# teamtomo/torch-motion-correction

Measured on AMD Instinct MI355X. Metric: frames/sec motion-corrected, 40×4k×4k fp32 stack, 1/2/4/8 MI355X, higher is better.
Workload: dtype f32; 1 GPU; 40-frame 4096x4096 fp32 movie, global rigid shift estimate+correct (estimate_global_motion -> correct_motion, frames + sum out), 1 stack per GPU per step, consecutive steps overlapped on two HIP streams; b_factor=500

## Files before the change

torch_motion_correction_amd/csrc/mc_fft.h:

```cpp
#pragma once
#include <type_traits>
#include "mc_common.h"

__device__ __forceinline__ int lpad(int i) { return i + (i >> 4); }
__host__ __device__ constexpr int lds_len(int n) { return n + (n >> 4) + 1; }

#define MC_SQRT1_2 0.70710678118654752440f

template <int DIR>
__device__ __forceinline__ void bfly2(cfloat* a) {
  cfloat t = a[0];
  a[0] = cadd(t, a[1]);
  a[1] = csub(t, a[1]);
}

template <int DIR>
__device__ __forceinline__ void bfly4(cfloat& a0, cfloat& a1, cfloat& a2, cfloat& a3) {
  cfloat t0 = cadd(a0, a2), t1 = csub(a0, a2);
  cfloat t2 = cadd(a1, a3), t3 = cmul_i<DIR>(csub(a1, a3));
  a0 = cadd(t0, t2);
  a1 = cadd(t1, t3);
  a2 = csub(t0, t2);
  a3 = csub(t1, t3);
}

template <int DIR>
__device__ __forceinline__ void bfly8(cfloat* a) {
  bfly4<DIR>(a[0], a[2], a[4], a[6]);
  bfly4<DIR>(a[1], a[3], a[5], a[7]);
  const float c = MC_SQRT1_2;
  cfloat o1, o2, o3;
  if (DIR < 0) {
    o1 = cmake(c * (a[3].x + a[3].y), c * (a[3].y - a[3].x));
    o3 = cmake(c * (a[7].y - a[7].x), -c * (a[7].x + a[7].y));
  } else {
    o1 = cmake(c * (a[3].x - a[3].y), c * (a[3].x + a[3].y));
    o3 = cmake(-c * (a[7].x + a[7].y), c * (a[7].x - a[7].y));
  }
  o2 = cmul_i<DIR>(a[5]);
  cfloat e0 = a[0], e1 = a[2], e2 = a[4], e3 = a[6], o0 = a[1];
  a[0] = cadd(e0, o0);
  a[4] = csub(e0, o0);
  a[1] = cadd(e1, o1);
  a[5] = csub(e1, o1);
  a[2] = cadd(e2, o2);
  a[6] = csub(e2, o2);
  a[3] = cadd(e3, o3);
  a[7] = csub(e3, o3);
}

template <int R, int DIR>
__device__ __forceinline__ void bfly(cfloat* a) {
  if constexpr (R == 8) bfly8<DIR>(a);
  else if constexpr (R == 4) bfly4<DIR>(a[0], a[1], a[2], a[3]);
  else bfly2<DIR>(a);
}

template <int N>
struct FftPlan {
  static constexpr int npass() {
    int n = N, p = 0;
    while (n > 1) {
      n /= (n >= 8 ? 8 : n);
      ++p;
    }
    return p;
  }
  static constexpr int radix(int pass) {
    int n = N, r = 1;
    for (int p = 0; p <= pass; ++p) {
      r = n >= 8 ? 8 : n;
      n /= r;
    }
    return r;
  }
  static constexpr int ns(int pass) {
    int n = 1;
    for (int p = 0; p < pass; ++p) n *= radix(p);
    return n;
  }
  static constexpr int iters(int pass) { return (N / radix(pass) + MC_WG - 1) / MC_WG; }
  static constexpr int max_iters() {
    int m = 1;
    for (int p = 0; p < npass(); ++p) m = iters(p) > m ? iters(p) : m;
    return m;
  }
};

__host__ __device__ constexpr int fft_threads(int n) {
  return (n / 8) < 64 ? 64 : ((n / 8) > MC_WG ? MC_WG : (n / 8));
}

template <int N>
struct FftTwiddles {
  static constexpr int P = FftPlan<N>::npass();
  static constexpr int NT = fft_threads(N);
  static constexpr int max_iters() {
    int m = 1;
    for (int p = 0; p < P; ++p) {
      const int it = (N / FftPlan<N>::radix(p) + NT - 1) / NT;
      m = it > m ? it : m;
    }
    return m;
  }
  cfloat w[P > 1 ? P - 1 : 1][max_iters()];
  template <int DIR>
  __device__ __forceinline__ void init(int lt, const cfloat* __restrict__ tw, int tw_stride) {
#pragma unroll
    for (int p = 1; p < P; ++p) {
      const int R = FftPlan<N>::radix(p), NS = FftPlan<N>::ns(p), NB = N / R;
      const int IT = (NB + NT - 1) / NT;
#pragma unroll
      for (int it = 0; it < IT; ++it) {
        const int j = lt + it * NT;
        const int k = j & (NS - 1);
        cfloat v = tw[(j < NB ? k : 0) * (N / (NS * R)) * tw_stride];
        if (DIR > 0) v.y = -v.y;
        w[p - 1][it] = v;
      }
    }
  }
};

template <int N, int PASS, int DIR, typename Load, typename Store>
__device__ __forceinline__ void fft_pass2(int lt, const FftTwiddles<N>& T, Load load, Store store) {
  constexpr int R = FftPlan<N>::radix(PASS);
  constexpr int NS = FftPlan<N>::ns(PASS);
  constexpr int NB = N / R;
  constexpr int NT = fft_threads(N);
  constexpr int IT = (NB + NT - 1) / NT;
  cfloat v[IT][R];
#pragma unroll
  for (int it = 0; it < IT; ++it) {
    const int j = lt + it * NT;
    if (NB % NT == 0 || j < NB) {
#pragma unroll
      for (int m = 0; m < R; ++m) v[it][m] = load(j + m * NB, it, m);
      if constexpr (NS > 1) {
        const cfloat w1 = T.w[PASS - 1][it];
        v[it][1] = cmul(v[it][1], w1);
        if constexpr (R >= 4) {
          const cfloat w2 = cmul(w1, w1), w3 = cmul(w2, w1);
          v[it][2] = cmul(v[it][2], w2);
          v[it][3] = cmul(v[it][3], w3);
          if constexpr (R == 8) {
            const cfloat w4 = cmul(w2, w2), w5 = cmul(w4, w1), w6 = cmul(w3, w3), w7 = cmul(w4, w3);
            v[it][4] = cmul(v[it][4], w4);
            v[it][5] = cmul(v[it][5], w5);
            v[it][6] = cmul(v[it][6], w6);
            v[it][7] = cmul(v[it][7], w7);
          }
        }
      }
      bfly<R, DIR>(v[it]);
      const int k = j & (NS - 1);
      const int base = (j - k) * R + k;
#pragma unroll
      for (int m = 0; m < R; ++m) store(base + m * NS, v[it][m]);
    }
  }
}

template <int N, int DIR, bool LAST_TO_FUNCTOR, int PASS, typename Load, typename Store>
__device__ __forceinline__ int fft_pp_rec(cfloat* l0, cfloat* l1, int s, int lt,
                                          const FftTwiddles<N>& T, Load load, Store store) {
  constexpr int P = FftPlan<N>::npass();
  cfloat* src = ((s + PASS + 1) & 1) ? l1 : l0;
  cfloat* dst = ((s + PASS) & 1) ? l1 : l0;
  auto lds_load = [src](int i, int, int) { return src[lpad(i)]; };
  auto lds_store = [dst](int i, cfloat v) { dst[lpad(i)] = v; };
  constexpr bool LAST = (PASS == P - 1);
  if constexpr (PASS == 0 && LAST) {
    if constexpr (LAST_TO_FUNCTOR) fft_pass2<N, PASS, DIR>(lt, T, load, store);
    else { fft_pass2<N, PASS, DIR>(lt, T, load, lds_store); __syncthreads(); }
    return (s + PASS) & 1;
  } else if constexpr (PASS == 0) {
    fft_pass2<N, PASS, DIR>(lt, T, load, lds_store);
    __syncthreads();
    return fft_pp_rec<N, DIR, LAST_TO_FUNCTOR, PASS + 1>(l0, l1, s, lt, T, load, store);
  } else if constexpr (LAST) {
    if constexpr (LAST_TO_FUNCTOR) {
      fft_pass2<N, PASS, DIR>(lt, T, lds_load, store);
      return (s + PASS + 1) & 1;
    } else {
      fft_pass2<N, PASS, DIR>(lt, T, lds_load, lds_store);
      __syncthreads();
      return (s + PASS) & 1;
    }
  } else {
    fft_pass2<N, PASS, DIR>(lt, T, lds_load, lds_store);
    __syncthreads();
    return fft_pp_rec<N, DIR, LAST_TO_FUNCTOR, PASS + 1>(l0, l1, s, lt, T, load, store);
  }
}

template <int N, int DIR, bool LAST_TO_FUNCTOR, typename Load, typename Store>
__device__ __forceinline__ int wg_fft_pp(cfloat* l0, cfloat* l1, int s, int lt,
                                         const FftTwiddles<N>& T, Load load, Store store) {
  return fft_pp_rec<N, DIR, LAST_TO_FUNCTOR, 0>(l0, l1, s, lt, T, load, store);
}

template <int N, int R, int NS, int DIR, bool SYNC_MID, bool SYNC_END, typename Load, typename Store>
__device__ __forceinline__ void fft_pass(int tid, const cfloat* __restrict__ tw, int tw_stride,
                                         Load load, Store store) {
  constexpr int NB = N / R;
  constexpr int IT = (NB + MC_WG - 1) / MC_WG;
  cfloat v[IT][R];
#pragma unroll
  for (int it = 0; it < IT; ++it) {
    const int j = tid + it * MC_WG;
    if (NB >= MC_WG || j < NB) {
#pragma unroll
      for (int m = 0; m < R; ++m) v[it][m] = load(j + m * NB);
      if constexpr (NS > 1) {
        const int k = j & (NS - 1);
        cfloat w1 = tw[k * (N / (NS * R)) * tw_stride];
        if (DIR > 0) w1.y = -w1.y;
        v[it][1] = cmul(v[it][1], w1);
        if constexpr (R >= 4) {
          cfloat w2 = cmul(w1, w1), w3 = cmul(w2, w1);
          v[it][2] = cmul(v[it][2], w2);
          v[it][3] = cmul(v[it][3], w3);
          if constexpr (R == 8) {
            cfloat w4 = cmul(w2, w2), w5 = cmul(w4, w1), w6 = cmul(w3, w3), w7 = cmul(w4, w3);
            v[it][4] = cmul(v[it][4], w4);
            v[it][5] = cmul(v[it][5], w5);
            v[it][6] = cmul(v[it][6], w6);
            v[it][7] = cmul(v[it][7], w7);
          }
        }
      }
      bfly<R, DIR>(v[it]);
    }
  }
  if (SYNC_MID) __syncthreads();
#pragma unroll
  for (int it = 0; it < IT; ++it) {
    const int j = tid + it * MC_WG;
    if (NB >= MC_WG || j < NB) {
      const int k = j & (NS - 1);
      const int base = (j - k) * R + k;
#pragma unroll
      for (int m = 0; m < R; ++m) store(base + m * NS, v[it][m]);
    }
  }
  if (SYNC_END) __syncthreads();
}

template <int N, int NS, int DIR, bool FIRST, bool FIRST_LDS = false, typename Load, typename Store>
__device__ __forceinline__ void fft_rec(cfloat* line, int tid, const cfloat* __restrict__ tw,
                                        int tw_stride, Load load, Store store) {
  constexpr int REM = N / NS;
  constexpr int R = REM >= 8 ? 8 : REM;
  constexpr bool LAST = (NS * R == N);
  auto lds_load = [line](int i) { return line[lpad(i)]; };
  auto lds_store = [line](int i, cfloat v) { line[lpad(i)] = v; };
  if constexpr (FIRST && LAST) {
    fft_pass<N, R, NS, DIR, FIRST_LDS, false>(tid, tw, tw_stride, load, store);
  } else if constexpr (FIRST) {
    fft_pass<N, R, NS, DIR, FIRST_LDS, true>(tid, tw, tw_stride, load, lds_store);
    fft_rec<N, NS * R, DIR, false>(line, tid, tw, tw_stride, load, store);
  } else if constexpr (LAST) {
    fft_pass<N, R, NS, DIR, true, false>(tid, tw, tw_stride, lds_load, store);
  } else {
    fft_pass<N, R, NS, DIR, true, true>(tid, tw, tw_stride, lds_load, lds_store);
    fft_rec<N, NS * R, DIR, false>(line, tid, tw, tw_stride, load, store);
  }
}

template <int N, int DIR, typename Load, typename Store>
__device__ __forceinline__ void wg_fft(cfloat* line, int tid, const cfloat* __restrict__ tw,
                                       int tw_stride, Load load, Store store) {
  fft_rec<N, 1, DIR, true>(line, tid, tw, tw_stride, load, store);
}

template <int N, int DIR, typename Load, typename Store>
__device__ __forceinline__ void wg_fft_inplace(cfloat* line, int tid, const cfloat* __restrict__ tw,
                                               int tw_stride, Load load, Store store) {
  fft_rec<N, 1, DIR, true, true>(line, tid, tw, tw_stride, load, store);
}

template <int DIR>
__device__ __forceinline__ void bfly3(cfloat* a) {
  const float s = 0.86602540378443864676f;
  const cfloat t1 = cadd(a[1], a[2]);
  const cfloat t2 = cmake(a[0].x - 0.5f * t1.x, a[0].y - 0.5f * t1.y);
  const cfloat d = cmul_i<DIR>(cscale(csub(a[1], a[2]), s));
  a[0] = cadd(a[0], t1);
  a[1] = cadd(t2, d);
  a[2] = csub(t2, d);
}

template <int DIR>
__device__ __forceinline__ void bfly5(cfloat* a) {
  const float c1 = 0.30901699437494742410f, c2 = -0.80901699437494742410f;
  const float s1 = 0.95105651629515357212f, s2 = 0.58778525229247312917f;
  const cfloat a1 = cadd(a[1], a[4]), a2 = cadd(a[2], a[3]);
  const cfloat b1 = csub(a[1], a[4]), b2 = csub(a[2], a[3]);
  const cfloat m1 = cmake(a[0].x + c1 * a1.x + c2 * a2.x, a[0].y + c1 * a1.y + c2 * a2.y);
  const cfloat m2 = cmake(a[0].x + c2 * a1.x + c1 * a2.x, a[0].y + c2 * a1.y + c1 * a2.y);
  const cfloat n1 = cmul_i<DIR>(cmake(s1 * b1.x + s2 * b2.x, s1 * b1.y + s2 * b2.y));
  const cfloat n2 = cmul_i<DIR>(cmake(s2 * b1.x - s1 * b2.x, s2 * b1.y - s1 * b2.y));
  a[0] = cadd(a[0], cadd(a1, a2));
  a[1] = cadd(m1, n1);
  a[4] = csub(m1, n1);
  a[2] = cadd(m2, n2);
  a[3] = csub(m2, n2);
}

constexpr double mc_cx_sincos(double x, bool want_sin) {
  double term = want_sin ? x : 1.0, sum = term;
  for (int k = want_sin ? 3 : 2; k < 70; k += 2) {
    term *= -x * x / (double)((k - 1) * k);
    sum += term;
  }
  return sum;
}
template <int R>
struct PrimeTab {
  float c[R], s[R];
  constexpr PrimeTab() : c{}, s{} {
    for (int j = 0; j < R; ++j) {
      const int jj = j <= R / 2 ? j : j - R;
      const double x = 6.283185307179586476925286766559 * (double)jj / (double)R;
      c[j] = (float)mc_cx_sincos(x, false);
      s[j] = (float)mc_cx_sincos(x, true);
    }
  }
};

template <int R, int DIR>
__device__ __forceinline__ void bfly_prime(cfloat* a) {
  constexpr int HF = (R - 1) / 2;
  constexpr PrimeTab<R> T{};
  cfloat s[HF], d[HF];
#pragma unroll
  for (int m = 1; m <= HF; ++m) {
    s[m - 1] = cadd(a[m], a[R - m]);
    d[m - 1] = csub(a[m], a[R - m]);
  }
  const cfloat x0 = a[0];
  cfloat tot = x0;
#pragma unroll
  for (int m = 0; m < HF; ++m) tot = cadd(tot, s[m]);
  a[0] = tot;
#pragma unroll
  for (int k = 1; k <= HF; ++k) {
    cfloat p = x0, q = cmake(0.f, 0.f);
#pragma unroll
    for (int m = 1; m <= HF; ++m) {
      const float c = T.c[(m * k) % R], sn = T.s[(m * k) % R];
      p.x = __builtin_fmaf(c, s[m - 1].x, p.x);
      p.y = __builtin_fmaf(c, s[m - 1].y, p.y);
      q.x = __builtin_fmaf(sn, d[m - 1].x, q.x);
      q.y = __builtin_fmaf(sn, d[m - 1].y, q.y);
    }
    const cfloat iq = cmul_i<DIR>(q);
    a[k] = cadd(p, iq);
    a[R - k] = csub(p, iq);
  }
}

template <int DIR>
__device__ __forceinline__ void bfly9(cfloat* a) {
  const float c1 = 0.76604444311897803520f, s1 = 0.64278760968653932632f;
  const float c2 = 0.17364817766693034885f, s2 = 0.98480775301220805937f;
  const float c4 = -0.93969262078590838405f, s4 = 0.34202014332566873304f;
  cfloat t[3][3];
#pragma unroll
  for (int n2 = 0; n2 < 3; ++n2) {
    cfloat u[3] = {a[n2], a[3 + n2], a[6 + n2]};
    bfly3<DIR>(u);
    t[n2][0] = u[0]; t[n2][1] = u[1]; t[n2][2] = u[2];
  }
  const float sg = DIR < 0 ? -1.f : 1.f;
  t[1][1] = cmul(t[1][1], cmake(c1, sg * s1));
  t[1][2] = cmul(t[1][2], cmake(c2, sg * s2));
  t[2][1] = cmul(t[2][1], cmake(c2, sg * s2));
  t[2][2] = cmul(t[2][2], cmake(c4, sg * s4));
#pragma unroll
  for (int k1 = 0; k1 < 3; ++k1) {
    cfloat u[3] = {t[0][k1], t[1][k1], t[2][k1]};
    bfly3<DIR>(u);
    a[k1] = u[0]; a[k1 + 3] = u[1]; a[k1 + 6] = u[2];
  }
}

template <int DIR>
__device__ __forceinline__ void bfly10(cfloat* a) {
  cfloat y0[5] = {a[0], a[2], a[4], a[6], a[8]};
  cfloat y1[5] = {a[5], a[7], a[9], a[1], a[3]};
  bfly5<DIR>(y0);
  bfly5<DIR>(y1);
#pragma unroll
  for (int k2 = 0; k2 < 5; ++k2) {
    a[(6 * k2) % 10] = cadd(y0[k2], y1[k2]);
    a[(5 + 6 * k2) % 10] = csub(y0[k2], y1[k2]);
  }
}

template <int R2, int DIR>
__device__ __forceinline__ void bfly_pfa3(cfloat* a) {
  constexpr int R = 3 * R2;
  constexpr int KA = R2 == 4 ? 4 : 16;
  cfloat y[3][R2];
#pragma unroll
  for (int n1 = 0; n1 < 3; ++n1) {
#pragma unroll
    for (int n2 = 0; n2 < R2; ++n2) y[n1][n2] = a[(R2 * n1 + 3 * n2) % R];
    bfly<R2, DIR>(y[n1]);
  }
#pragma unroll
  for (int k2 = 0; k2 < R2; ++k2) {
    cfloat u[3] = {y[0][k2], y[1][k2], y[2][k2]};
    bfly3<DIR>(u);
#pragma unroll
    for (int k1 = 0; k1 < 3; ++k1) a[(KA * k1 + 9 * k2) % R] = u[k1];
  }
}

template <int R, int DIR>
__device__ __forceinline__ void bfly_any(cfloat* a) {
  if constexpr (R == 12) bfly_pfa3<4, DIR>(a);
  else if constexpr (R == 24) bfly_pfa3<8, DIR>(a);
  else if constexpr (R == 9) bfly9<DIR>(a);
  else if constexpr (R == 10) bfly10<DIR>(a);
  else if constexpr (R == 5) bfly5<DIR>(a);
  else if constexpr (R == 3) bfly3<DIR>(a);
  else if constexpr (R == 7 || R == 11 || R == 13 || R == 31) bfly_prime<R, DIR>(a);
  else bfly<R, DIR>(a);
}

__host__ __device__ constexpr int smooth_radix(int rem) {
  return rem % 31 == 0 ? 31 : rem % 13 == 0 ? 13 : rem % 11 == 0 ? 11 : rem % 7 == 0 ? 7
       : rem == 24 ? 24 : rem == 12 ? 12 : rem % 8 == 0 ? 8
       : rem % 4 == 0 ? 4 : rem % 9 == 0 ? 9 : rem % 10 == 0 ? 10 : rem % 5 == 0 ? 5 : rem % 3 == 0 ? 3
       : rem % 2 == 0 ? 2 : 0;
}
__host__ __device__ constexpr bool is_smooth(int n) {
  while (n % 2 == 0) n /= 2;
  while (n % 3 == 0) n /= 3;
  while (n % 5 == 0) n /= 5;
  while (n % 7 == 0) n /= 7;
  while (n % 11 == 0) n /= 11;
  while (n % 13 == 0) n /= 13;
  while (n % 31 == 0) n /= 31;
  return n == 1;
}

template <int N, int R, int NS, int DIR, bool SYNC_MID, bool SYNC_END, int WG = MC_WG, typename Load, typename Store>
__device__ __forceinline__ void smooth_pass(int tid, const cfloat* __restrict__ tw, int tw_stride,
                                            Load load, Store store) {
  constexpr int NB = N / R;
  constexpr int IT = (NB + WG - 1) / WG;
  cfloat v[IT][R];
#pragma unroll
  for (int it = 0; it < IT; ++it) {
    const int j = tid + it * WG;
    if (j < NB) {
#pragma unroll
      for (int m = 0; m < R; ++m) v[it][m] = load(j + m * NB);
      if constexpr (NS > 1) {
        const int k = j % NS;
        if constexpr (R > 8) {
#pragma unroll
          for (int m = 1; m < R; ++m) {
            cfloat wm = tw[k * m * (N / (NS * R)) * tw_stride];
            if (DIR > 0) wm.y = -wm.y;
            v[it][m] = cmul(v[it][m], wm);
          }
        } else {
          cfloat w1 = tw[k * (N / (NS * R)) * tw_stride];
          if (DIR > 0) w1.y = -w1.y;
          cfloat wm = w1;
#pragma unroll
          for (int m = 1; m < R; ++m) {
            v[it][m] = cmul(v[it][m], wm);
            if (m + 1 < R) wm = cmul(wm, w1);
          }
        }
      }
      bfly_any<R, DIR>(v[it]);
    }
  }
  if (SYNC_MID) __syncthreads();
#pragma unroll
  for (int it = 0; it < IT; ++it) {
    const int j = tid + it * WG;
    if (j < NB) {
      const int k = j % NS;
      const int base = (j - k) * R + k;
#pragma unroll
      for (int m = 0; m < R; ++m) {
        if constexpr (std::is_invocable_v<Store, int, cfloat, int>) store(base + m * NS, v[it][m], it * R + m);
        else store(base + m * NS, v[it][m]);
      }
    }
  }
  if (SYNC_END) __syncthreads();
}

template <int N, int NS, int DIR, bool FIRST, bool FIRST_LDS = false, int WG = MC_WG, typename Load, typename Store>
__device__ __forceinline__ void smooth_rec(cfloat* line, int tid, const cfloat* __restrict__ tw,
                                           int tw_stride, Load load, Store store) {
  constexpr int R = smooth_radix(N / NS);
  static_assert(R > 0, "length is not of the form 2^a 3^b 5^c");
  constexpr bool LAST = (NS * R == N);
  auto lds_load = [line](int i) { return line[lpad(i)]; };
  auto lds_store = [line](int i, cfloat v) { line[lpad(i)] = v; };
  if constexpr (FIRST && LAST) {
    smooth_pass<N, R, NS, DIR, FIRST_LDS, false, WG>(tid, tw, tw_stride, load, store);
  } else if constexpr (FIRST) {
    smooth_pass<N, R, NS, DIR, FIRST_LDS, true, WG>(tid, tw, tw_stride, load, lds_store);
    smooth_rec<N, NS * R, DIR, false, false, WG>(line, tid, tw, tw_stride, load, store);
  } else if constexpr (LAST) {
    smooth_pass<N, R, NS, DIR, true, false, WG>(tid, tw, tw_stride, lds_load, store);
  } else {
    smooth_pass<N, R, NS, DIR, true, true, WG>(tid, tw, tw_stride, lds_load, lds_store);
    smooth_rec<N, NS * R, DIR, false, false, WG>(line, tid, tw, tw_stride, load, store);
  }
}

template <int N, int DIR, int WG = MC_WG, typename Load, typename Store>
__device__ __forceinline__ void wg_fft_any(cfloat* line, int tid, const cfloat* __restrict__ tw,
                                           int tw_stride, Load load, Store store) {
  if constexpr ((N & (N - 1)) == 0) {
    static_assert(WG == MC_WG, "power-of-two lines run on 256 threads");
    fft_rec<N, 1, DIR, true>(line, tid, tw, tw_stride, load, store);
  } else {
    smooth_rec<N, 1, DIR, true, false, WG>(line, tid, tw, tw_stride, load, store);
  }
}
template <int N, int DIR, int WG = MC_WG, typename Load, typename Store>
__device__ __forceinline__ void wg_fft_any_inplace(cfloat* line, int tid, const cfloat* __restrict__ tw,
                                                   int tw_stride, Load load, Store store) {
  if constexpr ((N & (N - 1)) == 0) {
    static_assert(WG == MC_WG, "power-of-two lines run on 256 threads");
    fft_rec<N, 1, DIR, true, true>(line, tid, tw, tw_stride, load, store);
  } else {
    smooth_rec<N, 1, DIR, true, true, WG>(line, tid, tw, tw_stride, load, store);
  }
}

template <int M, typename Load, typename Store>
__device__ __forceinline__ void wg_bluestein(cfloat* line, int tid, const cfloat* __restrict__ tw_m,
                                             const cfloat* __restrict__ chirp,
                                             const cfloat* __restrict__ bspec, int n, Load load,
                                             Store store, int keep = 0) {
  auto in1 = [&](int j) { return j < n ? cmul(load(j), chirp[j]) : cmake(0.f, 0.f); };
  auto out1 = [&](int j, cfloat v) { line[lpad(j)] = cmul(v, bspec[j]); };
  wg_fft_any<M, -1>(line, tid, tw_m, 1, in1, out1);
  __syncthreads();
  auto in2 = [&](int j) { return line[lpad(j)]; };
  auto out2 = [&](int p, cfloat v) {
    int k = p;
    if (keep > 0) {
      if (p > M - keep) {
        k = p - M + n;
        if (n & 1) v = cmake(-v.x, -v.y);
      } else if (p >= keep) {
        return;
      }
    }
    if (k < n) store(k, cmul(v, chirp[k]));
  };
  wg_fft_any_inplace<M, +1>(line, tid, tw_m, 1, in2, out2);
}

#include "mc_wave_fft.h"

struct R16Tw {
  wf2 a1, a2, a4, a8, b1, b2, b4, b8;
};
__device__ __forceinline__ R16Tw r16_twiddles(int tid, const cfloat* __restrict__ tw) {
  const int n3 = tid & 15;
  R16Tw t;
  t.a1 = wf_from(tw[tid]); t.a2 = wf_from(tw[2 * tid]); t.a4 = wf_from(tw[4 * tid]); t.a8 = wf_from(tw[8 * tid]);
  t.b1 = wf_from(tw[16 * n3]); t.b2 = wf_from(tw[32 * n3]); t.b4 = wf_from(tw[64 * n3]); t.b8 = wf_from(tw[128 * n3]);
  return t;
}

template <int DIR, int IN_KEEP, int OUT_KEEP, typename Load, typename Store>
__device__ __forceinline__ void wg_fft4096_r16_tw(cfloat* line_c, int tid, const R16Tw& TW, Load load, Store store);

template <int DIR, int IN_KEEP, int OUT_KEEP, typename Load, typename Store>
__device__ __forceinline__ void wg_fft4096_r16(cfloat* line_c, int tid, const cfloat* __restrict__ tw,
                                               Load load, Store store) {
  const R16Tw TW = r16_twiddles(tid, tw);
  wg_fft4096_r16_tw<DIR, IN_KEEP, OUT_KEEP>(line_c, tid, TW, load, store);
}

template <int DIR, int IN_KEEP, int OUT_KEEP, typename Load, typename Store>
__device__ __forceinline__ void wg_fft4096_r16_tw(cfloat* line_c, int tid, const R16Tw& TW, Load load, Store store) {
  wf2* line = reinterpret_cast<wf2*>(line_c);
  auto cj = [](wf2 v) { return DIR > 0 ? wf2{v.x, -v.y} : v; };
  wf2 a[16];
#pragma unroll
  for (int n1 = 0; n1 < 16; ++n1) {
    if (n1 < IN_KEEP || n1 >= 16 - IN_KEEP) a[n1] = cj(wf_from(load(n1, 256 * n1 + tid)));
    else a[n1] = wf2{0.f, 0.f};
  }
  if constexpr (IN_KEEP == 2) wf_dft16_lo2(a);
  else wf_dft16(a);
  {
    const wf2 w1 = TW.a1, w2 = TW.a2, w4 = TW.a4, w8 = TW.a8;
    const wf2 w3 = wf_cmul(w2, w1), w5 = wf_cmul(w4, w1), w6 = wf_cmul(w4, w2), w7 = wf_cmul(w4, w3);
    a[1] = wf_cmul(a[1], w1); a[2] = wf_cmul(a[2], w2); a[3] = wf_cmul(a[3], w3); a[4] = wf_cmul(a[4], w4);
    a[5] = wf_cmul(a[5], w5); a[6] = wf_cmul(a[6], w6); a[7] = wf_cmul(a[7], w7); a[8] = wf_cmul(a[8], w8);
    a[9] = wf_cmul(a[9], wf_cmul(w8, w1)); a[10] = wf_cmul(a[10], wf_cmul(w8, w2));
    a[11] = wf_cmul(a[11], wf_cmul(w8, w3)); a[12] = wf_cmul(a[12], wf_cmul(w8, w4));
    a[13] = wf_cmul(a[13], wf_cmul(w8, w5)); a[14] = wf_cmul(a[14], wf_cmul(w8, w6));
    a[15] = wf_cmul(a[15], wf_cmul(w8, w7));
  }
#pragma unroll
  for (int k1 = 0; k1 < 16; ++k1) line[k1 * 256 + (tid ^ (16 * (k1 & 1)))] = a[k1];
  __syncthreads();
  {
    const int k1 = tid >> 4, n3 = tid & 15;
#pragma unroll
    for (int n2 = 0; n2 < 16; ++n2) a[n2] = line[k1 * 256 + ((16 * n2 + n3) ^ (16 * (k1 & 1)))];
    __syncthreads();
    wf_dft16(a);
    const wf2 w1 = TW.b1, w2 = TW.b2, w4 = TW.b4, w8 = TW.b8;
    const wf2 w3 = wf_cmul(w2, w1), w5 = wf_cmul(w4, w1), w6 = wf_cmul(w4, w2), w7 = wf_cmul(w4, w3);
    a[1] = wf_cmul(a[1], w1); a[2] = wf_cmul(a[2], w2); a[3] = wf_cmul(a[3], w3); a[4] = wf_cmul(a[4], w4);
    a[5] = wf_cmul(a[5], w5); a[6] = wf_cmul(a[6], w6); a[7] = wf_cmul(a[7], w7); a[8] = wf_cmul(a[8], w8);
    a[9] = wf_cmul(a[9], wf_cmul(w8, w1)); a[10] = wf_cmul(a[10], wf_cmul(w8, w2));
    a[11] = wf_cmul(a[11], wf_cmul(w8, w3)); a[12] = wf_cmul(a[12], wf_cmul(w8, w4));
    a[13] = wf_cmul(a[13], wf_cmul(w8, w5)); a[14] = wf_cmul(a[14], wf_cmul(w8, w6));
    a[15] = wf_cmul(a[15], wf_cmul(w8, w7));
#pragma unroll
    for (int k2 = 0; k2 < 16; ++k2) line[k1 * 256 + k2 * 16 + (n3 ^ k1)] = a[k2];
  }
  __syncthreads();
  {
    const int k1 = tid & 15, k2 = tid >> 4;
#pragma unroll
    for (int n3 = 0; n3 < 16; ++n3) a[n3] = line[k1 * 256 + k2 * 16 + (n3 ^ k1)];
    wf_dft16(a);
#pragma unroll
    for (int k3 = 0; k3 < 16; ++k3)
      if (k3 < OUT_KEEP || k3 >= 16 - OUT_KEEP) {
        if constexpr (std::is_invocable_v<Store, int, int, cfloat>) store(k3, tid + 256 * k3, wf_to(cj(a[k3])));
        else store(tid + 256 * k3, wf_to(cj(a[k3])));
      }
  }
}
```

torch_motion_correction_amd/csrc/xc_search.hip:

```cpp
#include "xc_common.h"

__global__ void xc_search_init(int* __restrict__ best, int* __restrict__ gate, float* __restrict__ bounds,
                               int npairs, int nbounds, float* __restrict__ shift_table, int nshift) {
  const int i = blockIdx.x * blockDim.x + threadIdx.x;
  if (i < nbounds) bounds[i] = 0.f;
  if (i < nshift) shift_table[i] = 0.f;
  if (i < npairs) best[i] = (int)0x807fffffu;
  if (i == 0) gate[0] = 0;
}

__global__ void xc_far_needed(const float* __restrict__ bounds, const int* __restrict__ best,
                              float* __restrict__ part_val, int* __restrict__ part_idx,
                              int* __restrict__ need_full, int H, int RG, int near) {
  const int ngrp = H / RG;
  const int p = blockIdx.y;
  const int grp = near + blockIdx.x * blockDim.x + threadIdx.x;
  if (grp >= ngrp - near) return;
  float b = 0.f;
  for (int r = 0; r < RG; ++r) b = fmaxf(b, bounds[(int64_t)p * H + grp * RG + r]);
  b = b * 1.0001f + 1e-30f;
  part_val[(int64_t)p * ngrp + grp] = -INFINITY;
  part_idx[(int64_t)p * ngrp + grp] = 0x7fffffff;
  const int fb = __float_as_int(b);
  if ((fb >= 0 ? fb : fb ^ 0x7fffffff) >= best[p]) atomicOr(need_full, 1);
}



__global__ __launch_bounds__(256) void xc_row_bounds(const cfloat* __restrict__ T2,
                                                     float* __restrict__ bounds, int nkx, int H) {
  __shared__ float part[4][64];
  const int ly = threadIdx.x & 63, slice = threadIdx.x >> 6;
  const int y = blockIdx.x * 64 + ly;
  const int p = blockIdx.y;
  float b0 = 0.f, b1 = 0.f, b2 = 0.f, b3 = 0.f;
  if (y < H) {
    const cfloat* in = T2 + (int64_t)p * nkx * H + y;
    int kx = slice;
    for (; kx + 12 < nkx; kx += 16) {
      const cfloat v0 = in[(int64_t)kx * H], v1 = in[(int64_t)(kx + 4) * H];
      const cfloat v2 = in[(int64_t)(kx + 8) * H], v3 = in[(int64_t)(kx + 12) * H];
      b0 += (kx == 0 ? 1.f : 2.f) * sqrtf(v0.x * v0.x + v0.y * v0.y);
      b1 += 2.f * sqrtf(v1.x * v1.x + v1.y * v1.y);
      b2 += 2.f * sqrtf(v2.x * v2.x + v2.y * v2.y);
      b3 += 2.f * sqrtf(v3.x * v3.x + v3.y * v3.y);
    }
    for (; kx < nkx; kx += 4) {
      const cfloat v = in[(int64_t)kx * H];
      b0 += (kx == 0 ? 1.f : 2.f) * sqrtf(v.x * v.x + v.y * v.y);
    }
  }
  part[slice][ly] = (b0 + b1) + (b2 + b3);
  __syncthreads();
  if (slice == 0 && y < H)
    bounds[(int64_t)p * H + y] = (part[0][ly] + part[1][ly]) + (part[2][ly] + part[3][ly]);
}

template <int LOGN, int EPI>
__global__ __launch_bounds__(MC_WG) void xc_rows_inv(const cfloat* __restrict__ T2,
                                                     const float* __restrict__ bounds,
                                                     int* __restrict__ best,
                                                     float* __restrict__ part_val,
                                                     int* __restrict__ part_idx,
                                                     float* __restrict__ out_real,
                                                     const int64_t* __restrict__ out_off,
                                                     int64_t out_stride,
                                                     const cfloat* __restrict__ tw_row, XcGeom g,
                                                     int near, int phase, int compact,
                                                     const int* __restrict__ gate) {
  constexpr int N = 1 << LOGN;
  if (gate && gate[0] == 0) return;
  constexpr int NT = fft_threads(N), SG = MC_WG / NT;
  constexpr int R0 = FftPlan<N>::radix(0), NB0 = N / R0, IT0 = (NB0 + NT - 1) / NT;
  extern __shared__ __attribute__((aligned(16))) char smem[];
  const int tid = threadIdx.x;
  const int lt = tid & (NT - 1), sg = tid / NT;
  cfloat* l0 = reinterpret_cast<cfloat*>(smem) + sg * 2 * lds_len(N);
  cfloat* l1 = l0 + lds_len(N);
  cfloat* stg = reinterpret_cast<cfloat*>(smem) + SG * 2 * lds_len(N);
  const int p = blockIdx.y;
  const int RG = g.RG;
  const int ngrp = g.H / RG;
  int grp = blockIdx.x;
  if (EPI == 0) grp = phase == 0 ? ((int)blockIdx.x < near ? (int)blockIdx.x : ngrp - 2 * near + (int)blockIdx.x)
                                 : near + (int)blockIdx.x;
  if constexpr (EPI == 0) {
    if (phase == 1) {
      float b = 0.f;
      for (int r = 0; r < RG; ++r) b = fmaxf(b, bounds[(int64_t)p * g.H + grp * RG + r]);
      b = b * 1.0001f + 1e-30f;
      if (float_order(b) < __hip_atomic_load(&best[p], __ATOMIC_RELAXED, __HIP_MEMORY_SCOPE_AGENT)) {
        if (tid == 0) {
          part_val[(int64_t)p * ngrp + grp] = -INFINITY;
          part_idx[(int64_t)p * ngrp + grp] = 0x7fffffff;
        }
        return;
      }
    }
  }
  const int nstore = near * RG + (compact > 0 ? compact - 1 : 0);
  const int cstride = compact ? 2 * nstore : g.H;
  const int coff = (int)blockIdx.x < near ? (int)blockIdx.x * RG
                                          : nstore + (compact - 1) + ((int)blockIdx.x - near) * RG;
  const cfloat* in = T2 + (int64_t)p * g.nkx * cstride + (int64_t)(compact ? coff : grp * RG);
  for (int i0 = tid; i0 < g.nkx * RG; i0 += 8 * MC_WG) {
    cfloat v8[8];
#pragma unroll
    for (int u = 0; u < 8; ++u) {
      const int i = i0 + u * MC_WG;
      const int kx = i / RG, r = i - kx * RG;
      if (i < g.nkx * RG) v8[u] = in[(int64_t)kx * cstride + r];
    }
#pragma unroll
    for (int u = 0; u < 8; ++u) {
      const int i = i0 + u * MC_WG;
      const int kx = i / RG, r = i - kx * RG;
      if (i < g.nkx * RG) stg[kx * (RG + 1) + r] = v8[u];
    }
  }
  FftTwiddles<N> T;
  T.template init<+1>(lt, tw_row, 2);
  cfloat wk[IT0][R0];
#pragma unroll
  for (int it = 0; it < IT0; ++it)
#pragma unroll
    for (int q = 0; q < R0; ++q) {
      const int j = lt + it * NT;
      const int k = (NB0 % NT == 0 || j < NB0) ? j + q * NB0 : 0;
      cfloat w = tw_row[k];
      w.y = -w.y;
      wk[it][q] = w;
    }
  __syncthreads();
  float bv = -INFINITY;
  int bi = 0x7fffffff;
  int s = 0;
  for (int r = sg; r < RG; r += SG) {
    const int y = grp * RG + r;
    auto load = [&](int k, int it, int q) {
      const int km = N - k;
      cfloat xk = (k < g.nkx) ? stg[k * (RG + 1) + r] : cmake(0.f, 0.f);
      cfloat xm = (km < g.nkx) ? cconj(stg[km * (RG + 1) + r]) : cmake(0.f, 0.f);
      if (k == 0) {
        xk.y = 0.f;
        xm.y = 0.f;
      }
      const cfloat sm = cadd(xk, xm), d = csub(xk, xm);
      const cfloat wd = cmul(wk[it][q], d);
      return cmake(sm.x - wd.y, sm.y + wd.x);
    };
    int res;
    if constexpr (EPI == 0) {
      auto store = [&](int n, cfloat v) {
        const int flat = y * g.W + 2 * n;
        cand_merge(bv, bi, v.x, flat);
        cand_merge(bv, bi, v.y, flat + 1);
      };
      res = wg_fft_pp<N, +1, true>(l0, l1, s, lt, T, load, store);
    } else {
      float* orow = out_real + out_off[p] + (int64_t)y * out_stride;
      auto store = [&](int n, cfloat v) {
        orow[2 * n] = v.x;
        orow[2 * n + 1] = v.y;
      };
      res = wg_fft_pp<N, +1, true>(l0, l1, s, lt, T, load, store);
    }
    s = res ^ 1;
  }
  if constexpr (EPI == 0) {
    for (int off = 32; off > 0; off >>= 1) {
      const float ov = __shfl_down(bv, off);
      const int oi = __shfl_down(bi, off);
      cand_merge(bv, bi, ov, oi);
    }
    __shared__ float wv[MC_WG / 64];
    __shared__ int wi[MC_WG / 64];
    if ((tid & 63) == 0) {
      wv[tid >> 6] = bv;
      wi[tid >> 6] = bi;
    }
    __syncthreads();
    if (tid == 0) {
      for (int w = 1; w < MC_WG / 64; ++w) cand_merge(bv, bi, wv[w], wi[w]);
      part_val[(int64_t)p * ngrp + grp] = bv;
      part_idx[(int64_t)p * ngrp + grp] = bi;
      atomicMax(&best[p], float_order(bv));
    }
  }
}

__global__ void xc_peak_final(const float* __restrict__ part_val, const int* __restrict__ part_idx,
                              int ngrp, int H, int W, int* __restrict__ peaks,
                              float* __restrict__ shifts, const int* __restrict__ shift_rows) {
  const int p = blockIdx.x;
  float bv = -INFINITY;
  int bi = 0x7fffffff;
  for (int i = threadIdx.x; i < ngrp; i += blockDim.x)
    cand_merge(bv, bi, part_val[(int64_t)p * ngrp + i], part_idx[(int64_t)p * ngrp + i]);
  for (int off = 32; off > 0; off >>= 1) {
    const float ov = __shfl_down(bv, off);
    const int oi = __shfl_down(bi, off);
    cand_merge(bv, bi, ov, oi);
  }
  if (threadIdx.x == 0) {
    if (bi == 0x7fffffff) bi = 0;
    peaks[p] = bi;
    const int py = bi / W, px = bi - py * W;
    const int row = shift_rows ? shift_rows[p] : p;
    shifts[2 * row] = (float)(py <= H / 2 ? py : py - H);
    shifts[2 * row + 1] = (float)(px <= W / 2 ? px : px - W);
  }
}

template <int LOGN>
__global__ __launch_bounds__(MC_WG) void xc_peak_nbhd(const cfloat* __restrict__ T2,
                                                      const int* __restrict__ peaks,
                                                      float* __restrict__ nb,
                                                      const cfloat* __restrict__ tw_row, XcGeom g,
                                                      const cfloat* __restrict__ T2n,
                                                      const int* __restrict__ gate, int nstore) {
  constexpr int N = 1 << LOGN;
  __shared__ __attribute__((aligned(16))) cfloat line[lds_len(N)];
  const int tid = threadIdx.x;
  const int p = blockIdx.y, dy = (int)blockIdx.x - 1;
  const int pk = peaks[p];
  const int py = pk / g.W, px = pk - py * g.W;
  const int y = py + dy;
  float* o = nb + (int64_t)p * 9 + (dy + 1) * 3;
  if (y < 0 || y >= g.H) {
    if (tid < 3) o[tid] = __builtin_nanf("");
    return;
  }
  const cfloat* in = T2 + (int64_t)p * g.nkx * g.H + y;
  int64_t cs = g.H;
  if (T2n && gate[0] == 0) {
    const int yn = y < nstore ? y : y - (g.H - 2 * nstore);
    if (yn < 0 || yn >= 2 * nstore || (y >= nstore && y < g.H - nstore)) {
      if (tid < 3) o[tid] = __builtin_nanf("");
      return;
    }
    cs = 2 * nstore;
    in = T2n + (int64_t)p * g.nkx * cs + yn;
  }
  auto X = [&](int k) { return in[(int64_t)k * cs]; };
  auto load = [&](int k) {
    const int km = N - k;
    cfloat xk = (k < g.nkx) ? X(k) : cmake(0.f, 0.f);
    cfloat xm = (km < g.nkx) ? cconj(X(km)) : cmake(0.f, 0.f);
    if (k == 0) {
      xk.y = 0.f;
      xm.y = 0.f;
    }
    const cfloat s = cadd(xk, xm), d = csub(xk, xm);
    cfloat w = tw_row[k];
    w.y = -w.y;
    const cfloat wd = cmul(w, d);
    return cmake(s.x - wd.y, s.y + wd.x);
  };
  auto store = [&](int n, cfloat v) { line[lpad(n)] = v; };
  wg_fft<N, +1>(line, tid, tw_row, 2, load, store);
  __syncthreads();
  if (tid < 3) {
    const int x = px + tid - 1;
    float v = __builtin_nanf("");
    if (x >= 0 && x < g.W) {
      const cfloat z = line[lpad(x >> 1)];
      v = (x & 1) ? z.y : z.x;
    }
    o[tid] = v;
  }
}

void mc_launch_row_bounds(const cfloat* T2, float* bounds, int nkx, int H, int npairs, hipStream_t stream) {
  hipLaunchKernelGGL(xc_row_bounds, dim3((H + 63) / 64, npairs), dim3(256), 0, stream, T2, bounds, nkx, H);
}
void mc_launch_peak_final(const float* part_val, const int* part_idx, int ngrp, int H, int W, int* peaks,
                          float* shifts, const int* shift_rows, int npairs, hipStream_t stream) {
  hipLaunchKernelGGL(xc_peak_final, dim3(npairs), dim3(64), 0, stream, part_val, part_idx, ngrp, H, W, peaks, shifts,
                     shift_rows);
}

constexpr int XC_NEAR_GUARD = 8;

using RowsInvKernel = decltype(&xc_rows_inv<4, 0>);
template <int EPI>
static int rows_inv_kernel(const XcGeom& g, RowsInvKernel* k, size_t* lds) {
  *lds = rows_lds_bytes(g.W / 2, g);
  MC_DISPATCH_LOG(mc_ilog2(g.W) - 1, *k = xc_rows_inv<L, EPI>);
  return mc_dyn_lds(*k, *lds);
}
static void rows_argmax_launch(RowsInvKernel k, size_t lds, int ngroups, int npairs, const void* T2, const float* bounds,
                               int* best, float* part_val, int* part_idx, const void* tw_row, const XcGeom& g,
                               int near, int phase, int compact, const int* gate, hipStream_t stream) {
  hipLaunchKernelGGL(k, dim3(ngroups, npairs), dim3(MC_WG), lds, stream, (const cfloat*)T2, bounds, best, part_val,
                     part_idx, (float*)nullptr, (const int64_t*)nullptr, (int64_t)0, (const cfloat*)tw_row, g, near,
                     phase, compact, gate);
}

extern "C" {

int mc_xc_rows_inverse_argmax(const void* T2, float* part_val, int* part_idx, int* peaks,
                              float* shifts, const void* tw_row, int npairs, const mc_xc_geom* q,
                              void* stream) {
  XcGeom g;
  int rc = geom_from(q, &g, true, false);
  if (rc) return rc;
  if (!T2 || !part_val || !part_idx || !peaks || !shifts || !tw_row || npairs < 1)
    return MC_ERR_ARG;
  hipStream_t st = (hipStream_t)stream;
  RowsInvKernel k;
  size_t lds;
  if ((rc = rows_inv_kernel<0>(g, &k, &lds))) return rc;
  const int ngrp = g.H / g.RG;
  int* best = part_idx + (int64_t)npairs * ngrp;
  {
    const float ninf = -INFINITY;
    int pat;
    memcpy(&pat, &ninf, 4);
    pat = pat >= 0 ? pat : pat ^ 0x7fffffff;
    hipError_t e = hipMemsetD32Async((hipDeviceptr_t)best, pat, npairs, st);
    if (e != hipSuccess) return (int)e;
  }
  const int near = xc_near_groups(g), nfar = ngrp - 2 * near;
  float* bounds = part_val + (int64_t)npairs * ngrp;
  if (nfar > 0) mc_launch_row_bounds((const cfloat*)T2, bounds, g.nkx, g.H, npairs, st);
  if (near > 0)
    rows_argmax_launch(k, lds, 2 * near, npairs, T2, bounds, best, part_val, part_idx, tw_row, g, near, 0, 0, nullptr, st);
  if (nfar > 0)
    rows_argmax_launch(k, lds, nfar, npairs, T2, bounds, best, part_val, part_idx, tw_row, g, near, 1, 0, nullptr, st);
  rc = mc_check_launch();
  if (rc) return rc;
  mc_launch_peak_final(part_val, part_idx, ngrp, g.H, g.W, peaks, shifts, nullptr, npairs, st);
  return mc_check_launch();
}

int mc_xc_near_rows(const mc_xc_geom* q) {
  XcGeom g;
  int rc = geom_from(q, &g, true, true);
  if (rc) return rc;
  return xc_near_groups(g) * g.RG + XC_NEAR_GUARD;
}

int mc_xc_correlate_argmax(const void* S_cur, const int* cur_idx, const void* S_ref,
                           const int* ref_idx, void* T2_full, void* T2_near, float* part_val,
                           int* part_idx, int* peaks, float* shifts, const int* shift_rows,
                           int n_shift_rows, float* nb, const void* tw_col, const void* tw_row,
                           float scale, int npairs, const mc_xc_geom* q, void* stream) {
  XcGeom g;
  int rc = geom_from(q, &g, true, true);
  if (rc) return rc;
  if (!S_cur || !cur_idx || !S_ref || !ref_idx || !T2_full || !T2_near || !part_val || !part_idx ||
      !peaks || !shifts || !tw_col || !tw_row || npairs < 1)
    return MC_ERR_ARG;
  if (g.H < 1024) return MC_ERR_UNSUPPORTED;
  hipStream_t st = (hipStream_t)stream;
  RowsInvKernel k;
  size_t lds;
  if ((rc = rows_inv_kernel<0>(g, &k, &lds))) return rc;
  const int ngrp = g.H / g.RG;
  const int near = xc_near_groups(g);
  if (near < 1) return MC_ERR_UNSUPPORTED;
  const int nstore = near * g.RG + XC_NEAR_GUARD;
  if (nstore > 256) return MC_ERR_UNSUPPORTED;
  int* best = part_idx + (int64_t)npairs * ngrp;
  int* gate = best + npairs;
  float* bounds = part_val + (int64_t)npairs * ngrp;
  if (shift_rows && n_shift_rows < 1) return MC_ERR_ARG;
  hipLaunchKernelGGL(xc_search_init, dim3((npairs * g.H + 255) / 256), dim3(256), 0, st, best, gate, bounds,
                     npairs, npairs * g.H, shifts, shift_rows ? 2 * n_shift_rows : 0);
  rc = mc_launch_cols_inv_near((const cfloat*)S_cur, cur_idx, (const cfloat*)S_ref, ref_idx, (cfloat*)T2_near, bounds,
                               (const cfloat*)tw_col, scale, g, nstore, npairs, st);
  if (rc) return rc;
  rows_argmax_launch(k, lds, 2 * near, npairs, T2_near, bounds, best, part_val, part_idx, tw_row, g, near, 0,
                     1 + XC_NEAR_GUARD, nullptr, st);
  rc = mc_check_launch();
  if (rc) return rc;
  const int nfar = ngrp - 2 * near;
  if (nfar > 0) {
    hipLaunchKernelGGL(xc_far_needed, dim3((nfar + 63) / 64, npairs), dim3(64), 0, st,
                       (const float*)bounds, (const int*)best, part_val, part_idx, gate, g.H, g.RG, near);
    rc = mc_launch_cols_inv_gated((const cfloat*)S_cur, cur_idx, (const cfloat*)S_ref, ref_idx, (cfloat*)T2_full,
                                  (const cfloat*)tw_col, scale, g, gate, npairs, st);
    if (rc) return rc;
    rows_argmax_launch(k, lds, nfar, npairs, T2_full, bounds, best, part_val, part_idx, tw_row, g, near, 1, 0, gate, st);
    rc = mc_check_launch();
    if (rc) return rc;
  }
  mc_launch_peak_final(part_val, part_idx, ngrp, g.H, g.W, peaks, shifts, shift_rows, npairs, st);
  if (nb) {
    MC_DISPATCH_LOG(mc_ilog2(g.W) - 1, {
      hipLaunchKernelGGL(xc_peak_nbhd<L>, dim3(3, npairs), dim3(MC_WG), 0, st, (const cfloat*)T2_full,
                         (const int*)peaks, nb, (const cfloat*)tw_row, g, (const cfloat*)T2_near,
                         (const int*)gate, nstore);
    });
  }
  return mc_check_launch();
}

int mc_xc_rows_inverse_store(const void* T2, float* out, const int64_t* out_off,
                             int64_t out_stride, const void* tw_row, int nframes,
                             const mc_xc_geom* q, void* stream) {
  XcGeom g;
  int rc = geom_from(q, &g, true, false);
  if (rc) return rc;
  if (!T2 || !out || !out_off || !tw_row || nframes < 1) return MC_ERR_ARG;
  RowsInvKernel k;
  size_t lds;
  if ((rc = rows_inv_kernel<1>(g, &k, &lds))) return rc;
  hipLaunchKernelGGL(k, dim3(g.H / g.RG, nframes), dim3(MC_WG), lds, (hipStream_t)stream, (const cfloat*)T2,
                     (const float*)nullptr, (int*)nullptr, (float*)nullptr, (int*)nullptr, out, out_off, out_stride,
                     (const cfloat*)tw_row, g, 0, 0, 0, (const int*)nullptr);
  return mc_check_launch();
}

int mc_xc_peak_neighbourhood(const void* T2, const int* peaks, float* nb, const void* tw_row,
                             int npairs, const mc_xc_geom* q, void* stream) {
  XcGeom g;
  int rc = geom_from(q, &g, true, false);
  if (rc) return rc;
  if (!T2 || !peaks || !nb || !tw_row || npairs < 1) return MC_ERR_ARG;
  const int logn = mc_ilog2(g.W) - 1;
  dim3 grid(3, npairs);
  MC_DISPATCH_LOG(logn, {
    hipLaunchKernelGGL(xc_peak_nbhd<L>, grid, dim3(MC_WG), 0, (hipStream_t)stream,
                       (const cfloat*)T2, peaks, nb, (const cfloat*)tw_row, g, (const cfloat*)nullptr,
                       (const int*)nullptr, 0);
  });
  return mc_check_launch();
}

}
```

Before: 24700 frames/s.

## Add pruned near-row inverse FFT argmax kernel with finer row tiling

Adds a dedicated kernel for the near-row inverse row FFT and argmax. It stages four rows per block through LDS and uses a pruned first radix-8 butterfly that skips inputs known to be zero because only nkx spectral columns are live. Per-tile candidates are written into the bounds buffer, and the final peak reduction merges them in place of the near groups' partial results. This cuts wasted FFT arithmetic and exposes more blocks for the near region, at the cost of extra kernel variants and reuse of the bounds buffer as candidate storage.

After: 24440 frames/s. 0.99x the previous value.

```diff
diff --git a/torch_motion_correction_amd/csrc/mc_fft.h b/torch_motion_correction_amd/csrc/mc_fft.h
--- a/torch_motion_correction_amd/csrc/mc_fft.h
+++ b/torch_motion_correction_amd/csrc/mc_fft.h
@@ -25,9 +25,7 @@
 }
 
 template <int DIR>
-__device__ __forceinline__ void bfly8(cfloat* a) {
-  bfly4<DIR>(a[0], a[2], a[4], a[6]);
-  bfly4<DIR>(a[1], a[3], a[5], a[7]);
+__device__ __forceinline__ void bfly8_combine(cfloat* a) {
   const float c = MC_SQRT1_2;
   cfloat o1, o2, o3;
   if (DIR < 0) {
@@ -47,6 +45,40 @@
   a[6] = csub(e2, o2);
   a[3] = cadd(e3, o3);
   a[7] = csub(e3, o3);
+}
+
+template <int DIR>
+__device__ __forceinline__ void bfly8(cfloat* a) {
+  bfly4<DIR>(a[0], a[2], a[4], a[6]);
+  bfly4<DIR>(a[1], a[3], a[5], a[7]);
+  bfly8_combine<DIR>(a);
+}
+
+template <bool ZA, bool ZB>
+__device__ __forceinline__ cfloat cadd_z(cfloat a, cfloat b) {
+  return ZB ? (ZA ? cmake(0.f, 0.f) : a) : (ZA ? b : cadd(a, b));
+}
+template <bool ZA, bool ZB>
+__device__ __forceinline__ cfloat csub_z(cfloat a, cfloat b) {
+  return ZB ? (ZA ? cmake(0.f, 0.f) : a) : (ZA ? cmake(-b.x, -b.y) : csub(a, b));
+}
+template <int DIR, bool Z0, bool Z1, bool Z2, bool Z3>
+__device__ __forceinline__ void bfly4_z(cfloat& a0, cfloat& a1, cfloat& a2, cfloat& a3) {
+  constexpr bool ZE = Z0 && Z2, ZO = Z1 && Z3;
+  cfloat t0 = cadd_z<Z0, Z2>(a0, a2), t1 = csub_z<Z0, Z2>(a0, a2);
+  cfloat t2 = cadd_z<Z1, Z3>(a1, a3), t3 = cmul_i<DIR>(csub_z<Z1, Z3>(a1, a3));
+  a0 = cadd_z<ZE, ZO>(t0, t2);
+  a1 = cadd_z<ZE, ZO>(t1, t3);
+  a2 = csub_z<ZE, ZO>(t0, t2);
+  a3 = csub_z<ZE, ZO>(t1, t3);
+}
+template <int DIR, int KEEP>
+__device__ __forceinline__ void bfly8_lohi(cfloat* a) {
+  static_assert(KEEP >= 1 && KEEP <= 4, "a[0] and a[7] are always live");
+  constexpr bool Z1 = KEEP < 2, Z2 = KEEP < 3, Z3 = KEEP < 4;
+  bfly4_z<DIR, false, Z2, Z3, Z1>(a[0], a[2], a[4], a[6]);
+  bfly4_z<DIR, Z1, Z3, Z2, false>(a[1], a[3], a[5], a[7]);
+  bfly8_combine<DIR>(a);
 }
 
 template <int R, int DIR>
diff --git a/torch_motion_correction_amd/csrc/xc_search.hip b/torch_motion_correction_amd/csrc/xc_search.hip
--- a/torch_motion_correction_amd/csrc/xc_search.hip
+++ b/torch_motion_correction_amd/csrc/xc_search.hip
@@ -189,14 +189,142 @@
   }
 }
 
+constexpr int XC_NEAR_ROWS = 4;
+template <int LOGN, int KEEP>
+__global__ __launch_bounds__(MC_WG) void xc_rows_inv_near(const cfloat* __restrict__ T2n, int* __restrict__ best,
+                                                          float* __restrict__ near_cand,
+                                                          const cfloat* __restrict__ tw_row, XcGeom g, int near,
+                                                          int guard) {
+  constexpr int N = 1 << LOGN;
+  constexpr int NT = fft_threads(N), SG = MC_WG / NT;
+  constexpr int R0 = FftPlan<N>::radix(0), NB0 = N / R0, IT0 = (NB0 + NT - 1) / NT;
+  constexpr int ROWS = XC_NEAR_ROWS, NQ = KEEP < 4 ? 2 * KEEP : 8;
+  static_assert(R0 == 8 && FftPlan<N>::npass() > 1 && ROWS % SG == 0, "radix-8 first pass, then LDS passes");
+  extern __shared__ __attribute__((aligned(16))) char smem[];
+  const int tid = threadIdx.x;
+  const int lt = tid & (NT - 1), sg = tid / NT;
+  cfloat* l0 = reinterpret_cast<cfloat*>(smem) + sg * 2 * lds_len(N);
+  cfloat* l1 = l0 + lds_len(N);
+  cfloat* stg = reinterpret_cast<cfloat*>(smem) + SG * 2 * lds_len(N);
+  const int p = blockIdx.y;
+  const int nrow = near * g.RG, nstore = nrow + guard;
+  const int w0 = (int)blockIdx.x * ROWS;
+  const int y0 = w0 < nrow ? w0 : g.H - 2 * nrow + w0;
+  const int c0 = w0 < nrow ? w0 : nstore + guard + (w0 - nrow);
+  const int cstride = 2 * nstore;
+  auto q_of = [](int u) { return u < NQ / 2 ? u : 8 - NQ + u; };
+  cfloat wk[IT0][NQ];
+#pragma unroll
+  for (int it = 0; it < IT0; ++it)
+#pragma unroll
+    for (int u = 0; u < NQ; ++u) {
+      const int j = lt + it * NT;
+      const int k = (NB0 % NT == 0 || j < NB0) ? j + q_of(u) * NB0 : 0;
+      cfloat w = tw_row[k];
+      w.y = -w.y;
+      wk[it][u] = w;
+    }
+  FftTwiddles<N> T;
+  T.template init<+1>(lt, tw_row, 2);
+  const cfloat* in = T2n + (int64_t)p * g.nkx * cstride + c0;
+  for (int i0 = tid; i0 < g.nkx * ROWS; i0 += 8 * MC_WG) {
+    cfloat v8[8];
+#pragma unroll
+    for (int u = 0; u < 8; ++u) {
+      const int i = i0 + u * MC_WG;
+      const int kx = i / ROWS, r = i - kx * ROWS;
+      if (i < g.nkx * ROWS) v8[u] = in[(int64_t)kx * cstride + r];
+    }
+#pragma unroll
+    for (int u = 0; u < 8; ++u) {
+      const int i = i0 + u * MC_WG;
+      const int kx = i / ROWS, r = i - kx * ROWS;
+      if (i < g.nkx * ROWS) stg[kx * (ROWS + 1) + r] = v8[u];
+    }
+  }
+  __syncthreads();
+  float bv = -INFINITY;
+  int bi = 0x7fffffff;
+  int s = 0;
+  for (int r = sg; r < ROWS; r += SG) {
+    const int y = y0 + r;
+    auto load = [&](int k, cfloat w) {
+      const int km = N - k;
+      cfloat xk = (k < g.nkx) ? stg[k * (ROWS + 1) + r] : cmake(0.f, 0.f);
+      cfloat xm = (km < g.nkx) ? cconj(stg[km * (ROWS + 1) + r]) : cmake(0.f, 0.f);
+      if (k == 0) {
+        xk.y = 0.f;
+        xm.y = 0.f;
+      }
+      const cfloat sm = cadd(xk, xm), d = csub(xk, xm);
+      const cfloat wd = cmul(w, d);
+      return cmake(sm.x - wd.y, sm.y + wd.x);
+    };
+    {
+      cfloat* dst = (s & 1) ? l1 : l0;
+#pragma unroll
+      for (int it = 0; it < IT0; ++it) {
+        const int j = lt + it * NT;
+        if (NB0 % NT == 0 || j < NB0) {
+          cfloat v[8];
+#pragma unroll
+          for (int q = 0; q < 8; ++q) v[q] = cmake(0.f, 0.f);
+#pragma unroll
+          for (int u = 0; u < NQ; ++u) v[q_of(u)] = load(j + q_of(u) * NB0, wk[it][u]);
+          bfly8_lohi<+1, KEEP>(v);
+#pragma unroll
+          for (int m = 0; m < 8; ++m) dst[lpad(j * 8 + m)] = v[m];
+        }
+      }
+      __syncthreads();
+    }
+    auto store = [&](int n, cfloat v) {
+      const int flat = y * g.W + 2 * n;
+      cand_merge(bv, bi, v.x, flat);
+      cand_merge(bv, bi, v.y, flat + 1);
+    };
+    auto no_load = [](int, int, int) { return cmake(0.f, 0.f); };
+    const int res = fft_pp_rec<N, +1, true, 1>(l0, l1, s, lt, T, no_load, store);
+    s = res ^ 1;
+  }
+  for (int off = 32; off > 0; off >>= 1) {
+    const float ov = __shfl_down(bv, off);
+    const int oi = __shfl_down(bi, off);
+    cand_merge(bv, bi, ov, oi);
+  }
+  __shared__ float wv[MC_WG / 64];
+  __shared__ int wi[MC_WG / 64];
+  if ((tid & 63) == 0) {
+    wv[tid >> 6] = bv;
+    wi[tid >> 6] = bi;
+  }
+  __syncthreads();
+  if (tid == 0) {
+    for (int w = 1; w < MC_WG / 64; ++w) cand_merge(bv, bi, wv[w], wi[w]);
+    float* cand = near_cand + (int64_t)p * g.H + y0;
+    cand[0] = bv;
+    reinterpret_cast<int*>(cand)[1] = bi;
+    atomicMax(&best[p], float_order(bv));
+  }
+}
+
 __global__ void xc_peak_final(const float* __restrict__ part_val, const int* __restrict__ part_idx,
                               int ngrp, int H, int W, int* __restrict__ peaks,
-                              float* __restrict__ shifts, const int* __restrict__ shift_rows) {
+                              float* __restrict__ shifts, const int* __restrict__ shift_rows,
+                              const float* __restrict__ near_cand, int near, int RG, int rows) {
   const int p = blockIdx.x;
   float bv = -INFINITY;
   int bi = 0x7fffffff;
   for (int i = threadIdx.x; i < ngrp; i += blockDim.x)
-    cand_merge(bv, bi, part_val[(int64_t)p * ngrp + i], part_idx[(int64_t)p * ngrp + i]);
+    if (!near_cand || (i >= near && i < ngrp - near))
+      cand_merge(bv, bi, part_val[(int64_t)p * ngrp + i], part_idx[(int64_t)p * ngrp + i]);
+  if (near_cand) {
+    const int nrow = near * RG;
+    for (int w0 = threadIdx.x * rows; w0 < 2 * nrow; w0 += blockDim.x * rows) {
+      const float* cand = near_cand + (int64_t)p * H + (w0 < nrow ? w0 : H - 2 * nrow + w0);
+      cand_merge(bv, bi, cand[0], reinterpret_cast<const int*>(cand)[1]);
+    }
+  }
   for (int off = 32; off > 0; off >>= 1) {
     const float ov = __shfl_down(bv, off);
     const int oi = __shfl_down(bi, off);
@@ -277,7 +405,7 @@
 void mc_launch_peak_final(const float* part_val, const int* part_idx, int ngrp, int H, int W, int* peaks,
                           float* shifts, const int* shift_rows, int npairs, hipStream_t stream) {
   hipLaunchKernelGGL(xc_peak_final, dim3(npairs), dim3(64), 0, stream, part_val, part_idx, ngrp, H, W, peaks, shifts,
-                     shift_rows);
+                     shift_rows, (const float*)nullptr, 0, 0, 0);
 }
 
 constexpr int XC_NEAR_GUARD = 8;
@@ -295,6 +423,21 @@
   hipLaunchKernelGGL(k, dim3(ngroups, npairs), dim3(MC_WG), lds, stream, (const cfloat*)T2, bounds, best, part_val,
                      part_idx, (float*)nullptr, (const int64_t*)nullptr, (int64_t)0, (const cfloat*)tw_row, g, near,
                      phase, compact, gate);
+}
+
+using RowsNearKernel = decltype(&xc_rows_inv_near<4, 1>);
+static int rows_near_kernel(const XcGeom& g, RowsNearKernel* k, size_t* lds) {
+  *k = nullptr;
+  if (g.RG % XC_NEAR_ROWS) return MC_OK;
+  const int N = g.W / 2, keep = (g.nkx + N / 8 - 1) / (N / 8);
+  XcGeom tile = g;
+  tile.RG = XC_NEAR_ROWS;
+  *lds = rows_lds_bytes(N, tile);
+  MC_DISPATCH_LOG(mc_ilog2(g.W) - 1, {
+    *k = keep <= 1 ? xc_rows_inv_near<L, 1> : keep == 2 ? xc_rows_inv_near<L, 2>
+       : keep == 3 ? xc_rows_inv_near<L, 3> : xc_rows_inv_near<L, 4>;
+  });
+  return mc_dyn_lds(*k, *lds);
 }
 
 extern "C" {
@@ -371,8 +514,15 @@
   rc = mc_launch_cols_inv_near((const cfloat*)S_cur, cur_idx, (const cfloat*)S_ref, ref_idx, (cfloat*)T2_near, bounds,
                                (const cfloat*)tw_col, scale, g, nstore, npairs, st);
   if (rc) return rc;
-  rows_argmax_launch(k, lds, 2 * near, npairs, T2_near, bounds, best, part_val, part_idx, tw_row, g, near, 0,
-                     1 + XC_NEAR_GUARD, nullptr, st);
+  RowsNearKernel kn;
+  size_t lds_near;
+  if ((rc = rows_near_kernel(g, &kn, &lds_near))) return rc;
+  if (kn)
+    hipLaunchKernelGGL(kn, dim3(2 * near * g.RG / XC_NEAR_ROWS, npairs), dim3(MC_WG), lds_near, st,
+                       (const cfloat*)T2_near, best, bounds, (const cfloat*)tw_row, g, near, XC_NEAR_GUARD);
+  else
+    rows_argmax_launch(k, lds, 2 * near, npairs, T2_near, bounds, best, part_val, part_idx, tw_row, g, near, 0,
+                       1 + XC_NEAR_GUARD, nullptr, st);
   rc = mc_check_launch();
   if (rc) return rc;
   const int nfar = ngrp - 2 * near;
@@ -386,7 +536,9 @@
     rc = mc_check_launch();
     if (rc) return rc;
   }
-  mc_launch_peak_final(part_val, part_idx, ngrp, g.H, g.W, peaks, shifts, shift_rows, npairs, st);
+  hipLaunchKernelGGL(xc_peak_final, dim3(npairs), dim3(64), 0, st, (const float*)part_val, (const int*)part_idx, ngrp,
+                     g.H, g.W, peaks, shifts, shift_rows, (const float*)(kn ? bounds : nullptr), near, g.RG,
+                     XC_NEAR_ROWS);
   if (nb) {
     MC_DISPATCH_LOG(mc_ilog2(g.W) - 1, {
       hipLaunchKernelGGL(xc_peak_nbhd<L>, dim3(3, npairs), dim3(MC_WG), 0, st, (const cfloat*)T2_full,
```
